# matter-labs/era-boojum

Measured on NVIDIA H100. Metric: goldilocks_ntt_gelements_per_s, higher is better.
Workload: dtype u64

## Files before the change

### era_boojum_b200/csrc/capi.cu

```cuda
#include <cstdlib>
#include <cstring>
#include <memory>
#include "ctx.hpp"

namespace bj {
int32_t poseidon2_init_constants(bj_ctx* ctx);
}

namespace bj {
__global__ void field_selftest_kernel(u64 n, u64 seed, unsigned long long* mismatches) {
  const u64 i = (u64)blockIdx.x * blockDim.x + threadIdx.x;
  if (i >= n) return;
  auto next = [](u64& s) {
    s += 0x9E3779B97F4A7C15ull;
    u64 z = s;
    z = (z ^ (z >> 30)) * 0xBF58476D1CE4E5B9ull;
    z = (z ^ (z >> 27)) * 0x94D049BB133111EBull;
    return z ^ (z >> 31);
  };
  u64 st = seed + i * 0x632BE59BD9B4E019ull;
  const u64 edges[12] = {0, 1, gl::P - 1, gl::P, gl::P + 1, ~0ull, gl::EPS, gl::EPS + 1, 1ull << 63, gl::P - gl::EPS, 2, gl::P - 2};
  u64 a = next(st), b = next(st);
  if ((i & 7) == 0) a = edges[(i >> 3) % 12];
  if ((i & 15) < 2) b = edges[(i >> 4) % 12];
// ... 2 lines not shown
    a = (1ull << ((i >> 3) & 63)) + (((i >> 9) & 3) == 1 ? 1 : 0) - (((i >> 9) & 3) == 2 ? 1 : 0);
    const unsigned sel = (unsigned)(i >> 11) & 7;
    u64 lo = r & 0xffffffffull, hi = r >> 32;
    if (sel & 1) lo = (sel & 4) ? 0xffffffffull : 0;
    if (sel & 2) hi = (sel & 4) ? 0xffffffffull : 0;
    b = (hi << 32) | lo;
  }
  if ((i & 63) == 5) {
    a = edges[(i >> 6) % 12];
    b = edges[(i >> 6) / 12 % 12];
  }
  unsigned bad = 0;
  if (gl::mul(a, b) != gl::mul_c(a, b)) bad++;
  if (gl::canon(gl::mul_lazy(a, b)) != gl::mul_c(a, b)) bad++;
  const u64 bc = gl::canon(b);
  if (gl::canon(gl::add(a, bc)) != gl::canon(gl::add_c(a, bc))) bad++;
  if (gl::canon(gl::sub(a, bc)) != gl::canon(gl::sub_c(a, bc))) bad++;
  if (gl::canon(gl::add(a, gl::P)) != gl::canon(a)) bad++;
  if (gl::canon(gl::sub(a, gl::P)) != gl::canon(a)) bad++;
  if (gl::mul(a, b) >= gl::P) bad++;
  if (bad) atomicAdd(mismatches, (unsigned long long)bad);
}
}

namespace bj {
static cudaMemPool_t private_pool(int device) {
  cudaMemPoolProps props = {};
  props.allocType = cudaMemAllocationTypePinned;
  props.handleTypes = cudaMemHandleTypeNone;
  props.location.type = cudaMemLocationTypeDevice;
  props.location.id = device;
  cudaMemPool_t pool = nullptr;
  if (cudaMemPoolCreate(&pool, &props) != cudaSuccess) {
    cudaGetLastError();
    return nullptr;
  }
  uint64_t keep = ~0ull;
  cudaMemPoolSetAttribute(pool, cudaMemPoolAttrReleaseThreshold, &keep);
  return pool;
}

int32_t ctx_new_lane(bj_ctx* parent, bj_ctx** out) {
  std::unique_ptr<bj_ctx> lane(new bj_ctx());
  lane->device = parent->device;
  lane->sm_count = parent->sm_count;
  lane->l2_persist_bytes = parent->l2_persist_bytes;
  lane->l2_window_max = parent->l2_window_max;
  lane->ntt_use_v2 = parent->ntt_use_v2;
  lane->ntt_col_fastest = parent->ntt_col_fastest;
  lane->ntt_max_tile_log = parent->ntt_max_tile_log;
  lane->ntt_pass1_w = parent->ntt_pass1_w;
  lane->ntt_chunk_mb = parent->ntt_chunk_mb;
  lane->ntt_full_pow = parent->ntt_full_pow;
  lane->gate_peephole = parent->gate_peephole;
  lane->gate_points_per_thread = parent->gate_points_per_thread;
  lane->ntt_l2_persist = 0;
  lane->ntt_bulk = parent->ntt_bulk;
  lane->memory_limit = parent->memory_limit;
  lane->allow_recompute_plan = parent->allow_recompute_plan;
  lane->max_row_blocks = parent->max_row_blocks;
  lane->own_twiddles = false;
  BJ_CUDA(parent, cudaStreamCreateWithFlags(&lane->stream, cudaStreamNonBlocking));
  lane->own_stream = true;
  lane->pool = private_pool(parent->device);
  {
    std::lock_guard<std::mutex> lock(parent->tables_mu);
    const cudaError_t e = cudaStreamSynchronize(parent->stream);
    if (e != cudaSuccess) {
      cudaStreamDestroy(lane->stream);
      if (lane->pool) cudaMemPoolDestroy(lane->pool);
      BJ_FAIL(parent, BJ_ERR_CUDA, std::string("bj_ctx_create_lane: cudaStreamSynchronize: ") + cudaGetErrorString(e));
    }
    lane->parent = parent;
    parent->lanes++;
  }
  *out = lane.release();
  return BJ_OK;
}
}

using namespace bj;

extern "C" {

int32_t bj_selftest_field(bj_ctx* ctx, uint64_t n, uint64_t seed, uint64_t* h_mismatches) {
  bj::DeviceGuard device_guard(ctx);
  if (!ctx || !h_mismatches) return BJ_ERR_INVALID_ARG;
  *h_mismatches = 0;
  if (n == 0) return BJ_OK;
  struct Counter {
    unsigned long long* d = nullptr;
    ~Counter() {
      if (d) cudaFree(d);
    }
  } c;
  BJ_CUDA(ctx, cudaMalloc(&c.d, sizeof(unsigned long long)));
  BJ_CUDA(ctx, cudaMemsetAsync(c.d, 0, sizeof(unsigned long long), ctx->stream));
  field_selftest_kernel<<<(unsigned)((n + 255) / 256), 256, 0, ctx->stream>>>(n, seed, c.d);
  BJ_LAUNCH_CHECK(ctx);
  unsigned long long h = 0;
  BJ_CUDA(ctx, cudaMemcpyAsync(&h, c.d, sizeof(h), cudaMemcpyDeviceToHost, ctx->stream));
  BJ_CUDA(ctx, cudaStreamSynchronize(ctx->stream));
  *h_mismatches = h;
  return BJ_OK;
}

// ... 2 lines not shown
const char* bj_status_string(int32_t s) {
  switch (s) {
    case BJ_OK: return "ok";
    case BJ_ERR_INVALID_ARG: return "invalid argument";
    case BJ_ERR_CUDA: return "CUDA error";
    case BJ_ERR_NO_DEVICE: return "no CUDA device (this library has no CPU fallback)";
    case BJ_ERR_OOM: return "out of device memory";
    case BJ_ERR_UNSUPPORTED: return "unsupported";
    default: return "unknown status";
  }
}

static int env_int(const char* name, int dflt) {
  const char* v = getenv(name);
  return v && *v ? atoi(v) : dflt;
}

int32_t bj_ctx_create(int32_t device, void* stream, bj_ctx** out_ctx) {
  if (!out_ctx) return BJ_ERR_INVALID_ARG;
  *out_ctx = nullptr;
  int count = 0;
  if (cudaGetDeviceCount(&count) != cudaSuccess || count == 0) {
    cudaGetLastError();
    return BJ_ERR_NO_DEVICE;
  }
  if (device < 0 || device >= count) return BJ_ERR_INVALID_ARG;
  bj_ctx* ctx = new bj_ctx();
  ctx->device = device;
  bj::DeviceGuard device_guard(ctx);
  {
    int cur = -1;
    if (cudaGetDevice(&cur) != cudaSuccess || cur != device) {
      cudaGetLastError();
      delete ctx;
      return BJ_ERR_CUDA;
    }
  }
  ctx->stream = (cudaStream_t)stream;
  cudaDeviceProp prop;
  if (cudaGetDeviceProperties(&prop, device) == cudaSuccess) {
    ctx->sm_count = prop.multiProcessorCount;
    ctx->l2_persist_bytes = std::min<size_t>((size_t)prop.l2CacheSize * 3 / 8, (size_t)prop.persistingL2CacheMaxSize);
    ctx->l2_window_max = (size_t)prop.accessPolicyMaxWindowSize;
  }
  ctx->ntt_max_tile_log = env_int("BJ_NTT_MAX_TILE_LOG", 13);
  ctx->gate_points_per_thread = env_int("BJ_GATE_POINTS_PER_THREAD", 0);
  ctx->gate_peephole = env_int("BJ_GATE_PEEPHOLE", 15);
  if (ctx->ntt_max_tile_log < 8) ctx->ntt_max_tile_log = 8;
  if (ctx->ntt_max_tile_log > 14) ctx->ntt_max_tile_log = 14;
  ctx->ntt_pass1_w = env_int("BJ_NTT_PASS1_W", -1);
  ctx->ntt_use_v2 = env_int("BJ_NTT_V2", 1);
  ctx->ntt_col_fastest = env_int("BJ_NTT_COL_FASTEST", -1);
  ctx->ntt_full_pow = env_int("BJ_NTT_FULL_POW", 1);
  ctx->ntt_bulk = env_int("BJ_NTT_BULK", 0);
  ctx->ntt_l2_persist = env_int("BJ_NTT_L2_PERSIST", 1);
  ctx->ntt_chunk_mb = env_int("BJ_NTT_CHUNK_MB", 0);
  ctx->pool = private_pool(device);
  int32_t st = poseidon2_init_constants(ctx);
  if (st != BJ_OK) {
    if (ctx->pool) cudaMemPoolDestroy(ctx->pool);
    delete ctx;
    return st;
  }
  *out_ctx = ctx;
  return BJ_OK;
}

int32_t bj_ctx_destroy(bj_ctx* ctx) {
  if (!ctx) return BJ_OK;
  bj::DeviceGuard device_guard(ctx);
  if (const uint32_t alive = ctx->lanes.load())
    BJ_FAIL(ctx, BJ_ERR_INVALID_ARG, "bj_ctx_destroy: " + std::to_string(alive) + " lane(s) of this context are alive: destroy them first");
  if (ctx->parent) {
    std::lock_guard<std::mutex> lock(ctx->parent->tables_mu);
    if (ctx->witness_sets)
      BJ_FAIL(ctx, BJ_ERR_INVALID_ARG, "bj_ctx_destroy: " + std::to_string(ctx->witness_sets) + " witness slot set(s) of this lane are alive: free them first");
  }
  cudaStreamSynchronize(ctx->stream);
  if (ctx->witness_stream) {
    cudaStreamSynchronize(ctx->witness_stream);
    cudaStreamDestroy(ctx->witness_stream);
  }
  if (ctx->own_twiddles) {
    if (ctx->tw_fwd) cudaFree(ctx->tw_fwd);
    if (ctx->tw_inv) cudaFree(ctx->tw_inv);
  }
  for (auto& e : ctx->pow_cache) {
    cudaFree(e.lo);
    cudaFree(e.hi);
    if (e.full) cudaFree(e.full);
  }
  for (void* p : ctx->tables_retired) cudaFree(p);
  if (ctx->pow_best) cudaFree(ctx->pow_best);
  if (ctx->gate_program) cudaFree(ctx->gate_program);
  if (ctx->pool) cudaMemPoolDestroy(ctx->pool);
  if (ctx->scratch) cudaFree(ctx->scratch);
  if (ctx->ptr_table) cudaFree(ctx->ptr_table);
  if (ctx->param_arena) cudaFree(ctx->param_arena);
  if (ctx->host_ring) cudaFree(ctx->host_ring);
  if (ctx->copy_streams_ready) {
    cudaStreamDestroy(ctx->h2d_stream);
    cudaStreamDestroy(ctx->d2h_stream);
    for (int i = 0; i < 3; i++) {
      cudaEventDestroy(ctx->ev_up[i]);
      cudaEventDestroy(ctx->ev_done[i]);
      cudaEventDestroy(ctx->ev_down[i]);
    }
  }
  if (ctx->own_stream) cudaStreamDestroy(ctx->stream);
  if (ctx->parent) {
    std::lock_guard<std::mutex> lock(ctx->parent->tables_mu);
    ctx->parent->lanes--;
  }
  delete ctx;
  return BJ_OK;
}

int32_t bj_ctx_set_stream(bj_ctx* ctx, void* stream) {
  bj::DeviceGuard device_guard(ctx);
  if (!ctx) return BJ_ERR_INVALID_ARG;
  if (ctx->parent) BJ_FAIL(ctx, BJ_ERR_INVALID_ARG, "bj_ctx_set_stream: a lane keeps the stream it was created with");
  BJ_CUDA(ctx, cudaStreamSynchronize(ctx->stream));
  ctx->stream = (cudaStream_t)stream;
  return BJ_OK;
}

int32_t bj_ctx_set_coset_shard(bj_ctx* ctx, uint32_t rank, uint32_t world, uint32_t log_lde) {
  bj::DeviceGuard device_guard(ctx);
  if (!ctx) return BJ_ERR_INVALID_ARG;
  if (world == 0 || (world & (world - 1)) || rank >= world || log_lde > 16 || world > (1u << log_lde))
    BJ_FAIL(ctx, BJ_ERR_INVALID_ARG, "bj_ctx_set_coset_shard: world must be a power of two <= the LDE factor and rank < world");
  uint32_t ls = 0;
  while ((1u << ls) < world) ls++;
  ctx->shard_log_lde = log_lde;
  ctx->shard.first = rank;
  ctx->shard.log_stride = ls;
  ctx->shard.log_split = 0;
  return BJ_OK;
}

int32_t bj_ctx_set_domain_shard(bj_ctx* ctx, uint32_t rank, uint32_t world, uint32_t log_lde) {
  bj::DeviceGuard device_guard(ctx);
  if (!ctx) return BJ_ERR_INVALID_ARG;
  if (world == 0 || (world & (world - 1)) || rank >= world || log_lde > 16 || world > (8u << log_lde))
// ... 124 lines not shown
```

### era_boojum_b200/csrc/ctx.hpp

```cpp
#pragma once
#include <cuda_runtime.h>
#include <stdint.h>
#include <algorithm>
#include <atomic>
#include <mutex>
#include <string>
#include <vector>
#include "../../include/boojum_b200.h"
#include "gl64.cuh"

namespace bj {
using gl::u64;
using gl::u32;

struct PowTab {
  u64 coset;
  int log_n;
  u64 scale;
  int split;
  u64* lo;
  u64* hi;
  u64* full;
};

struct CosetShard {
  uint32_t first = 0;
  uint32_t log_stride = 0;
  uint32_t log_split = 0;
  __host__ __device__ __forceinline__ u64 global_index(u64 t_loc, int log_coset_len) const {
    if (log_stride == 0) return t_loc;
    const int lu = log_coset_len - (int)log_split;
    const u64 i = t_loc & ((1ull << lu) - 1);
    const u64 k = t_loc >> lu;
    return ((((k << log_stride) | first)) << lu) | i;
  }
  __host__ __device__ __forceinline__ u64 unit_of(u64 rank, u64 k) const { return (k << log_stride) | rank; }
  __host__ __device__ __forceinline__ u64 global_unit(u64 k) const { return unit_of(first, k); }
  __host__ __device__ __forceinline__ u64 local_units(u64 cosets) const {
    const u64 stride = 1ull << log_stride, group = cosets << log_split;
    if (group >= stride) return group >> log_stride;
    return first < group ? 1 : 0;
  }
  __host__ __device__ __forceinline__ u64 local_points(u64 cosets, int log_coset_len) const {
    return local_units(cosets) << (log_coset_len - (int)log_split);
  }
  __host__ __device__ __forceinline__ u32 owner(u64 t, int log_coset_len) const {
    return (u32)((t >> (log_coset_len - (int)log_split)) & ((1ull << log_stride) - 1));
  }
  __host__ __device__ __forceinline__ u64 owner_index(u64 t, int log_coset_len) const {
    const int lu = log_coset_len - (int)log_split;
    return (((t >> lu) >> log_stride) << lu) | (t & ((1ull << lu) - 1));
  }
  __host__ u64 unit_shift(u64 u, u32 log_n, u32 log_lde) const {
    const u64 j = u >> log_split, p = u & ((1ull << log_split) - 1);
    u64 jr = 0, pr = 0;
    for (u32 b = 0; b < log_lde; b++) jr |= ((j >> b) & 1) << (log_lde - 1 - b);
    for (u32 b = 0; b < log_split; b++) pr |= ((p >> b) & 1) << (log_split - 1 - b);
    u64 s = gl::mul(gl::MULT_GEN, gl::pow(gl::omega(log_n + log_lde), jr));
    if (log_split) s = gl::mul(s, gl::pow(gl::omega(log_n), pr));
    return s;
  }
  __host__ static CosetShard window(uint32_t log_units, uint32_t u, uint32_t log_split = 0) {
    CosetShard w;
    w.first = u;
    w.log_stride = log_units;
    w.log_split = log_split;
    return w;
  }
};

}

struct bj_comm;

struct bj_ctx {
  int device = 0;
  bj_comm* comm = nullptr;
  cudaStream_t stream = nullptr;
  bool own_stream = false;
  std::string last_error;
  bj::u64* tw_fwd = nullptr;
  bj::u64* tw_inv = nullptr;
  int tw_log = 0;
  std::vector<bj::PowTab> pow_cache;
  size_t pow_full_bytes = 0;
  void* scratch = nullptr;
  size_t scratch_bytes = 0;
  void* ptr_table = nullptr;
  size_t ptr_table_bytes = 0;
  bool copy_streams_ready = false;
  cudaStream_t h2d_stream = nullptr, d2h_stream = nullptr;
  cudaEvent_t ev_up[3] = {}, ev_done[3] = {}, ev_down[3] = {};
  void* host_ring = nullptr;
  size_t host_ring_bytes = 0;
  cudaStream_t witness_stream = nullptr;
  uint32_t witness_sets = 0;
  uint64_t witness_set_bytes = 0;
  uint32_t lane_witness_sets = 0;
  uint64_t lane_witness_set_bytes = 0;
  void* param_arena = nullptr;
  size_t param_off = 0;
  uint64_t launches = 0;
  int sm_count = 132;
  bool ntt_attr_set = false;
  std::vector<void*> attr_done;
  int ntt_use_v2 = 1;
  int ntt_col_fastest = -1;
  int ntt_max_tile_log = 13;
  int ntt_pass1_w = -1;
  int ntt_chunk_mb = 0;
  int ntt_full_pow = 1;
  uint32_t one = 1;
  int gate_peephole = 15;
  int gate_points_per_thread = 0;
  int ntt_l2_persist = 1;
  bool l2_limit_set = false;
  size_t l2_persist_bytes = 0;
  size_t l2_window_max = 0;
  int ntt_bulk = 0;
  cudaMemPool_t pool = nullptr;
  bj::CosetShard shard;
  uint32_t shard_log_lde = 0;
  uint64_t memory_limit = 0;
  bool allow_recompute_plan = false;
  bool allow_sharded_recompute_plan = false;
  uint32_t max_row_blocks = 1;
  unsigned long long* pow_best = nullptr;
  void* gate_program = nullptr;
  size_t gate_program_bytes = 0;
  bj_ctx* parent = nullptr;
  std::atomic<uint32_t> lanes{0};
  std::mutex tables_mu;
  std::vector<void*> tables_retired;
  bool own_twiddles = true;
  std::vector<const bj_setup*> setups;
};

#define BJ_FAIL(ctx, code, msg)          \
  do {                                   \
    if (ctx) (ctx)->last_error = (msg);  \
    return (code);                       \
  } while (0)

#define BJ_CUDA(ctx, expr)                                                                      \
  do {                                                                                          \
    cudaError_t _e = (expr);                                                                    \
    if (_e != cudaSuccess) {                                                                    \
      if (ctx) (ctx)->last_error = std::string(#expr) + ": " + cudaGetErrorString(_e);          \
      return BJ_ERR_CUDA;                                                                       \
    }                                                                                           \
  } while (0)

#define BJ_TRY(expr)                 \
  do {                               \
    int32_t _s = (expr);             \
    if (_s != BJ_OK) return _s;      \
  } while (0)

#define BJ_LAUNCH_CHECK(ctx)                                                              \
  do {                                                                                    \
    (ctx)->launches++;                                                                    \
    cudaError_t _e = cudaGetLastError();                                                  \
    if (_e != cudaSuccess) {                                                              \
      (ctx)->last_error = std::string("kernel launch: ") + cudaGetErrorString(_e);        \
// ... 35 lines not shown
```

### era_boojum_b200/csrc/ntt.cu

```cuda
#include <algorithm>
#include <cstdlib>
#include "ctx.hpp"
#include "ntt.cuh"
#include "ntt_v2.cuh"

namespace bj {

using gl::u32;

__device__ __forceinline__ int phys(int e) { return e + (e >> 4); }

__device__ __forceinline__ u64 scale_factor(const NttPass& p, u64 idx) {
  if (p.scale_mode == SCALE_CONST) return p.scale_const;
  if (p.scale_mode == SCALE_FULL) return __ldg(p.pw_full + idx);
  u64 lo = __ldg(p.pw_lo + (idx & ((1ull << p.pw_split) - 1)));
  u64 hi = __ldg(p.pw_hi + (idx >> p.pw_split));
  return gl::mul(lo, hi);
}

template <int RS>
__device__ __forceinline__ void stage_compute(u64 (&x)[16], const u64* __restrict__ tab, u32 pfx) {
#pragma unroll
  for (int q = 0; q < RS; q++) {
    const int bit = 1 << (3 - q);
// ... 9 lines not shown
    }
  }
}

__global__ void __launch_bounds__(512) ntt_pass_kernel(const NttPass p) {
  extern __shared__ u64 sm[];
  const int t = p.t, w = p.w, LOG_E = t + w;
  const int E = 1 << LOG_E, W = 1 << w;
  const int tid = threadIdx.x, nthr = blockDim.x;
  const u64 tile = blockIdx.x;
  const u64* __restrict__ src = p.src + (u64)blockIdx.y * p.src_col_stride;
  u64* __restrict__ dst = p.dst + (u64)blockIdx.y * p.dst_col_stride;
  const int m = p.log_n, r0 = p.r0;
  const bool do_scale = p.scale_mode != SCALE_NONE;

  u64 base = 0, S = 1;
  u32 hi = 0;
  if (p.kind == PASS_TILE) {
    const int lo_bits = m - r0 - t;
    const int groups_log = lo_bits - w;
    S = 1ull << lo_bits;
    hi = (u32)(tile >> groups_log);
    const u64 lo0 = (tile & ((1ull << groups_log) - 1)) << w;
    base = ((u64)hi << (m - r0)) + lo0;
    for (int e = tid; e < E; e += nthr) {
      const int row = e >> w, col = e & (W - 1);
      const u64 gi = base + (u64)row * S + col;
      u64 v = src[gi];
      if (do_scale && p.scale_on_load) v = gl::mul(v, scale_factor(p, gi));
      sm[phys(e)] = v;
    }
  } else {
    for (int idx = tid; idx < E; idx += nthr) {
      const int col = idx >> t, row = idx & ((1 << t) - 1);
      const u32 k1 = (u32)(tile << w) + col;
      const u32 blk = r0 ? (__brev(k1) >> (32 - r0)) : 0u;
      const u64 gi = ((u64)blk << t) + row;
      u64 v = src[gi];
      if (do_scale && p.scale_on_load) v = gl::mul(v, scale_factor(p, gi));
      sm[phys(row * W + col)] = v;
    }
  }
  __syncthreads();

  int done = 0;
  int rs = t & 3;
  if (rs == 0) rs = 4;
  const int nvt = E >> 4;
  while (done < t) {
    const int b_lo = t - done - rs;
    const int pp = b_lo + w - (4 - rs);
    for (int q = tid; q < nvt; q += nthr) {
      const int e0 = ((q >> pp) << (pp + 4)) | (q & ((1 << pp) - 1));
      u32 hq = hi;
      if (p.kind != PASS_TILE) {
        const u32 k1 = (u32)(tile << w) + (e0 & (W - 1));
        hq = r0 ? (__brev(k1) >> (32 - r0)) : 0u;
      }
      const u32 pfx = (hq << (LOG_E - pp - 4)) | (u32)(q >> pp);
      u64 x[16];
#pragma unroll
      for (int j = 0; j < 16; j++) x[j] = sm[phys(e0 | (j << pp))];
      switch (rs) {
        case 1: stage_compute<1>(x, p.tab, pfx); break;
        case 2: stage_compute<2>(x, p.tab, pfx); break;
        case 3: stage_compute<3>(x, p.tab, pfx); break;
        default: stage_compute<4>(x, p.tab, pfx); break;
      }
#pragma unroll
      for (int j = 0; j < 16; j++) sm[phys(e0 | (j << pp))] = x[j];
    }
    __syncthreads();
    done += rs;
    rs = 4;
  }

  if (p.kind == PASS_TILE) {
    for (int e = tid; e < E; e += nthr) {
      const int row = e >> w, col = e & (W - 1);
      const u64 gi = base + (u64)row * S + col;
      u64 v = sm[phys(e)];
      if (do_scale && !p.scale_on_load) v = gl::mul(v, scale_factor(p, gi));
      if (p.canon_out) v = gl::canon(v);
      dst[gi] = v;
    }
  } else {
    for (int idx = tid; idx < E; idx += nthr) {
      const int col = idx & (W - 1);
      const u32 kappa = (u32)(idx >> w);
      const u32 rho = t ? (__brev(kappa) >> (32 - t)) : 0u;
      u64 v = sm[phys((int)rho * W + col)];
      const u64 k1 = (tile << w) + col;
      const u64 go = k1 + ((u64)kappa << r0);
      if (do_scale && !p.scale_on_load) v = gl::mul(v, scale_factor(p, go));
      if (p.canon_out) v = gl::canon(v);
      dst[go] = v;
    }
  }
}

__global__ void ntt_small_kernel(u64* data, u64 col_stride, u32 n_cols, int log_n, const u64* __restrict__ tab,
                                 u64 coset_or_inv, u64 n_inv, int inverse) {
  const u32 c = blockIdx.x * blockDim.x + threadIdx.x;
  if (c >= n_cols) return;
  u64* a = data + (u64)c * col_stride;
  const int n = 1 << log_n;
  u64 x[8];
// ... 4 lines not shown
      x[i] = gl::mul(x[i], s);
      s = gl::mul(s, coset_or_inv);
    }
  }
  int pairs = n / 2, groups = 1, dist = n / 2;
  while (groups < n) {
    for (int k = 0; k < groups; k++) {
      const u64 s = tab[k];
      for (int j = k * pairs * 2; j < k * pairs * 2 + pairs; j++) {
        const u64 u = x[j], v = gl::mul(x[j + dist], s);
        x[j + dist] = gl::canon(gl::sub(u, v));
        x[j] = gl::canon(gl::add(u, v));
      }
    }
    pairs /= 2;
    groups *= 2;
    dist /= 2;
  }
  if (inverse) {
    u64 y[8];
    for (int i = 0; i < n; i++) y[log_n ? (__brev((u32)i) >> (32 - log_n)) : 0] = x[i];
    u64 s = n_inv;
    for (int i = 0; i < n; i++) {
      x[i] = gl::mul(y[i], s);
      s = gl::mul(s, coset_or_inv);
    }
  }
  for (int i = 0; i < n; i++) a[i] = gl::canon(x[i]);
}

struct PowSquares {
  u64 sq[33];
};

__global__ void twiddle_table_kernel(u64* tab, u32 count, int bits, PowSquares ps) {
  const u32 k = blockIdx.x * blockDim.x + threadIdx.x;
  if (k >= count) return;
  const u32 e = bits ? (__brev(k) >> (32 - bits)) : 0u;
  u64 r = 1;
  for (int b = 0; b < bits; b++)
    if ((e >> b) & 1) r = gl::mul(r, ps.sq[b]);
  tab[k] = gl::canon(r);
}

__global__ void pow_table_kernel(u64* out, u32 count, int bits, PowSquares ps, u64 scale) {
  const u32 i = blockIdx.x * blockDim.x + threadIdx.x;
  if (i >= count) return;
  u64 r = scale;
  for (int b = 0; b < bits; b++)
    if ((i >> b) & 1) r = gl::mul(r, ps.sq[b]);
  out[i] = gl::canon(r);
}

__global__ void bitreverse_kernel(u64* data, u64 col_stride, int log_n) {
  const u64 i = (u64)blockIdx.x * blockDim.x + threadIdx.x;
  if (i >= (1ull << log_n)) return;
  u64* a = data + (u64)blockIdx.y * col_stride;
  const u64 j = __brevll(i) >> (64 - log_n);
  if (i < j) {
    const u64 t = a[i];
    a[i] = a[j];
    a[j] = t;
  }
}


int32_t ensure_scratch(bj_ctx* ctx, size_t bytes) {
  if (ctx->scratch_bytes >= bytes) return BJ_OK;
  if (ctx->scratch) {
    BJ_CUDA(ctx, cudaStreamSynchronize(ctx->stream));
    BJ_CUDA(ctx, cudaFree(ctx->scratch));
    ctx->scratch = nullptr;
    ctx->scratch_bytes = 0;
  }
  cudaError_t e = cudaMalloc(&ctx->scratch, bytes);
  if (e != cudaSuccess) {
    cudaGetLastError();
    BJ_FAIL(ctx, BJ_ERR_OOM, "scratch allocation failed");
  }
  ctx->scratch_bytes = bytes;
  return BJ_OK;
}

static PowSquares make_squares(u64 w) {
  PowSquares ps;
  for (int b = 0; b < 33; b++) {
    ps.sq[b] = w;
    w = gl::sqr(w);
  }
  return ps;
}

static int32_t release_retired(bj_ctx* owner) {
  if (owner->tables_retired.empty() || owner->lanes.load() > 0) return BJ_OK;
  BJ_CUDA(owner, cudaStreamSynchronize(owner->stream));
  for (void* p : owner->tables_retired) cudaFree(p);
  owner->tables_retired.clear();
  owner->pow_full_bytes = 0;
  for (const auto& e : owner->pow_cache)
    if (e.full) owner->pow_full_bytes += sizeof(u64) << e.log_n;
  return BJ_OK;
}

int32_t ensure_twiddles(bj_ctx* ctx, int log_n) {
  if (log_n < 1) log_n = 1;
  if (log_n > 32) BJ_FAIL(ctx, BJ_ERR_INVALID_ARG, "log_n > 32 (two-adicity of the field)");
  if (ctx->tw_log >= log_n) return BJ_OK;
  if (ctx->parent && !ctx->own_twiddles) {
    bj_ctx* p = ctx->parent;
    std::lock_guard<std::mutex> lock(p->tables_mu);
    if (p->tw_log >= log_n) {
      ctx->tw_fwd = p->tw_fwd;
      ctx->tw_inv = p->tw_inv;
      ctx->tw_log = p->tw_log;
      return BJ_OK;
    }
    ctx->tw_fwd = ctx->tw_inv = nullptr;
    ctx->tw_log = 0;
    ctx->own_twiddles = true;
  }
  std::unique_lock<std::mutex> lock(ctx->tables_mu, std::defer_lock);
  if (!ctx->parent) {
    lock.lock();
    BJ_TRY(release_retired(ctx));
  }
  if (ctx->tw_fwd) {
    BJ_CUDA(ctx, cudaStreamSynchronize(ctx->stream));
    if (ctx->lanes.load() > 0) {
      ctx->tables_retired.push_back(ctx->tw_fwd);
      ctx->tables_retired.push_back(ctx->tw_inv);
    } else {
      cudaFree(ctx->tw_fwd);
      cudaFree(ctx->tw_inv);
    }
    ctx->tw_fwd = ctx->tw_inv = nullptr;
    ctx->tw_log = 0;
  }
  const u32 count = 1u << (log_n - 1);
  u64 *fwd = nullptr, *inv = nullptr;
  BJ_CUDA(ctx, cudaMalloc(&fwd, sizeof(u64) * count));
  BJ_CUDA(ctx, cudaMalloc(&inv, sizeof(u64) * count));
  const u64 w = gl::omega(log_n);
  const u32 blocks = (count + 255) / 256;
  twiddle_table_kernel<<<blocks, 256, 0, ctx->stream>>>(fwd, count, log_n - 1, make_squares(w));
  BJ_LAUNCH_CHECK(ctx);
  twiddle_table_kernel<<<blocks, 256, 0, ctx->stream>>>(inv, count, log_n - 1, make_squares(gl::inv(w)));
  BJ_LAUNCH_CHECK(ctx);
  if (ctx->lanes.load() > 0) BJ_CUDA(ctx, cudaStreamSynchronize(ctx->stream));
  ctx->tw_fwd = fwd;
  ctx->tw_inv = inv;
  ctx->tw_log = log_n;
  return BJ_OK;
}

__global__ void __launch_bounds__(256) pow_full_kernel(u64* __restrict__ full, u64 n, const u64* __restrict__ lo,
                                                        const u64* __restrict__ hi, int split) {
  const u64 i = (u64)blockIdx.x * blockDim.x + threadIdx.x;
  if (i >= n) return;
  full[i] = gl::mul(__ldg(lo + (i & ((1ull << split) - 1))), __ldg(hi + (i >> split)));
}

static constexpr size_t POW_FULL_BUDGET = (size_t)3 << 30;
static int32_t get_pow_tables(bj_ctx* ctx, u64 c, int log_n, u64 scale, PowTab* out) {
  bj_ctx* owner = ctx->parent ? ctx->parent : ctx;
  std::lock_guard<std::mutex> lock(owner->tables_mu);
  if (owner == ctx) BJ_TRY(release_retired(ctx));
  for (auto& e : owner->pow_cache)
    if (e.coset == c && e.log_n == log_n && e.scale == scale) {
      *out = e;
      return BJ_OK;
    }
  const bool shared = owner->lanes.load() > 0;
  if (owner->pow_cache.size() >= 64) {
    BJ_CUDA(ctx, cudaStreamSynchronize(ctx->stream));
    for (auto& e : owner->pow_cache) {
      if (shared) {
        owner->tables_retired.insert(owner->tables_retired.end(), {(void*)e.lo, (void*)e.hi});
        if (e.full) owner->tables_retired.push_back(e.full);
        continue;
      }
      cudaFree(e.lo);
      cudaFree(e.hi);
      if (e.full) cudaFree(e.full);
    }
    owner->pow_cache.clear();
    if (!shared) owner->pow_full_bytes = 0;
  }
  PowTab pt;
  pt.coset = c;
  pt.log_n = log_n;
  pt.scale = scale;
  pt.split = log_n / 2;
  const u32 nlo = 1u << pt.split, nhi = 1u << (log_n - pt.split);
  BJ_CUDA(ctx, cudaMalloc(&pt.lo, sizeof(u64) * nlo));
  BJ_CUDA(ctx, cudaMalloc(&pt.hi, sizeof(u64) * nhi));
  pow_table_kernel<<<(nlo + 255) / 256, 256, 0, ctx->stream>>>(pt.lo, nlo, pt.split, make_squares(c), 1);
  BJ_LAUNCH_CHECK(ctx);
  const u64 chi = gl::pow(c, 1ull << pt.split);
  pow_table_kernel<<<(nhi + 255) / 256, 256, 0, ctx->stream>>>(pt.hi, nhi, log_n - pt.split, make_squares(chi),
                                                                gl::canon(scale));
  BJ_LAUNCH_CHECK(ctx);
  pt.full = nullptr;
  const size_t full_bytes = sizeof(u64) << log_n;
  if (ctx->ntt_full_pow && log_n >= 8 && owner->pow_full_bytes + full_bytes <= POW_FULL_BUDGET &&
      cudaMalloc(&pt.full, full_bytes) == cudaSuccess) {
    const u64 n = 1ull << log_n;
    pow_full_kernel<<<(unsigned)((n + 255) / 256), 256, 0, ctx->stream>>>(pt.full, n, pt.lo, pt.hi, pt.split);
    BJ_LAUNCH_CHECK(ctx);
    owner->pow_full_bytes += full_bytes;
  } else {
    cudaGetLastError();
    pt.full = nullptr;
  }
  if (shared) BJ_CUDA(ctx, cudaStreamSynchronize(ctx->stream));
  owner->pow_cache.push_back(pt);
  *out = pt;
  return BJ_OK;
}

int32_t get_pow_tables_public(bj_ctx* ctx, u64 c, int log_n, u64 scale, PowTab* out) { return get_pow_tables(ctx, c, log_n, scale, out); }

static constexpr int NTT_MAX_PASSES = 6;

struct Plan {
  int n_pass;
  int t[NTT_MAX_PASSES];
  int w[NTT_MAX_PASSES];
};

static bool make_plan(const bj_ctx* ctx, int m, bool transpose_last, Plan* out) {
  Plan& pl = *out;
  pl = Plan{};
  const int MAXE = ctx->ntt_max_tile_log;
  if (m <= 12) {
    pl.n_pass = 1;
    pl.t[0] = m;
    pl.w[0] = 0;
    return true;
  }
  const int TL = transpose_last ? MAXE - 2 : MAXE;
  const int TM = MAXE - 2;
  int t_last = std::min(TL, std::max((m + 1) / 2, m - 10));
  int rest = m - t_last;
  int n_front = (rest + TM - 1) / TM;
  pl.n_pass = n_front + 1;
  if (pl.n_pass > NTT_MAX_PASSES) return false;
  int r0 = 0;
  for (int i = 0; i < n_front; i++) {
    int ti = rest / (n_front - i);
    rest -= ti;
    int wi = ctx->ntt_pass1_w >= 0 ? ctx->ntt_pass1_w : std::max(2, std::min(5, MAXE - ti));
    wi = std::min(wi, MAXE - ti);
    wi = std::min(wi, m - r0 - ti);
    if (ti + wi < 4) wi = 4 - ti;
    pl.t[i] = ti;
    pl.w[i] = wi;
    r0 += ti;
  }
  pl.t[n_front] = t_last;
  pl.w[n_front] = transpose_last ? std::min(std::min(MAXE - t_last, 5), r0) : 0;
  return true;
}

static constexpr u32 MAX_GRID_Y = 65535;

template <typename F>
static int32_t launch_column_slices(bj_ctx* ctx, const NttPass& p, u32 n_cols, F&& fn) {
  for (u32 c0 = 0; c0 < n_cols; c0 += std::min(MAX_GRID_Y, n_cols - c0)) {
    NttPass ps = p;
    ps.src = p.src + (u64)c0 * p.src_col_stride;
    ps.dst = p.dst + (u64)c0 * p.dst_col_stride;
    fn(ps, std::min(MAX_GRID_Y, n_cols - c0));
    BJ_LAUNCH_CHECK(ctx);
  }
// ... 23 lines not shown
    bool col_fastest;
    if (ctx->ntt_col_fastest >= 0) {
      col_fastest = (ctx->ntt_col_fastest >> (is_last ? 1 : 0)) & 1;
    } else {
      const bool big_table = p.scale_mode == SCALE_FULL && (sizeof(u64) << p.log_n) > ctx->l2_persist_bytes;
      col_fastest = is_last || big_table;
    }
    if (p.kind == PASS_TILE && !bulk && col_fastest && tiles * n_cols <= 0x7fffffffull) {
      NttPass ps = p;
      ps.n_cols = n_cols;
      v2.fn<<<(unsigned)(tiles * n_cols), v2.threads, v2.smem, ctx->stream>>>(ps);
      BJ_LAUNCH_CHECK(ctx);
      return BJ_OK;
    }
    return launch_column_slices(ctx, p, n_cols, [&](const NttPass& ps, u32 cols) {
      v2.fn<<<dim3((unsigned)tiles, cols, 1), v2.threads, v2.smem, ctx->stream>>>(ps);
    });
  }
  const int threads = std::max(32, std::min(512, (1 << LOG_E) >> 4));
  const size_t smem = sizeof(u64) * ((size_t)(1 << LOG_E) + ((size_t)(1 << LOG_E) >> 4) + 1);
  if (!ctx->ntt_attr_set) {
    BJ_CUDA(ctx, cudaFuncSetAttribute(ntt_pass_kernel, cudaFuncAttributeMaxDynamicSharedMemorySize, 200 * 1024));
    BJ_CUDA(ctx, cudaFuncSetAttribute(ntt_pass_kernel, cudaFuncAttributePreferredSharedMemoryCarveout,
                                      cudaSharedmemCarveoutMaxShared));
    ctx->ntt_attr_set = true;
  }
  return launch_column_slices(ctx, p, n_cols, [&](const NttPass& ps, u32 cols) {
    ntt_pass_kernel<<<dim3((unsigned)tiles, cols, 1), threads, smem, ctx->stream>>>(ps);
  });
}

static int32_t run_transform(bj_ctx* ctx, const u64* src, u64 src_stride, u64* dst, u64 dst_stride, int m,
                             u32 n_cols, u64 coset, bool inverse, u64* scratch, u64 scratch_stride) {
  BJ_TRY(ensure_twiddles(ctx, m));
  const u64* tab = inverse ? ctx->tw_inv : ctx->tw_fwd;
  coset = gl::canon(coset);
  if (m < 4) {
    if (src != dst || src_stride != dst_stride) {
      for (u32 c = 0; c < n_cols; c++)
        BJ_CUDA(ctx, cudaMemcpyAsync(dst + c * dst_stride, src + c * src_stride, sizeof(u64) << m,
                                     cudaMemcpyDeviceToDevice, ctx->stream));
    }
    const u64 n_inv = gl::inv((u64)1 << m);
    ntt_small_kernel<<<(n_cols + 63) / 64, 64, 0, ctx->stream>>>(dst, dst_stride, n_cols, m, tab,
                                                                 inverse ? gl::inv(coset) : coset, n_inv, inverse);
    BJ_LAUNCH_CHECK(ctx);
    return BJ_OK;
  }
  Plan pl;
  if (!make_plan(ctx, m, inverse, &pl)) BJ_FAIL(ctx, BJ_ERR_UNSUPPORTED, "NTT plan needs more passes than NTT_MAX_PASSES");
  PowTab pt{};
  int scale_mode = SCALE_NONE;
  u64 scale_const = 1;
  if (!inverse) {
    if (coset != 1) {
      BJ_TRY(get_pow_tables(ctx, coset, m, 1, &pt));
      scale_mode = SCALE_POW;
    }
  } else {
    const u64 n_inv = gl::inv((u64)1 << m);
    if (coset != 1) {
      BJ_TRY(get_pow_tables(ctx, gl::inv(coset), m, n_inv, &pt));
      scale_mode = SCALE_POW;
    } else {
      scale_mode = SCALE_CONST;
      scale_const = n_inv;
    }
  }
  const u64* cur_src = src;
  u64 cur_src_stride = src_stride;
  int r0 = 0;
  for (int i = 0; i < pl.n_pass; i++) {
    const bool first = i == 0, last = i == pl.n_pass - 1;
    NttPass p{};
    p.tab = tab;
    p.log_n = m;
    p.r0 = r0;
    p.t = pl.t[i];
    p.w = pl.w[i];
    p.kind = (inverse && last) ? PASS_TRANSPOSE_LAST : PASS_TILE;
    p.src = cur_src;
    p.src_col_stride = cur_src_stride;
    if (inverse && pl.n_pass > 1) {
      const int remaining = pl.n_pass - 1 - i;
      const bool to_dst = (remaining % 2) == 0;
      p.dst = to_dst ? dst : scratch;
      p.dst_col_stride = to_dst ? dst_stride : scratch_stride;
      if (last && p.dst == p.src) BJ_FAIL(ctx, BJ_ERR_INVALID_ARG, "internal: in-place transpose pass");
    } else {
      p.dst = dst;
      p.dst_col_stride = dst_stride;
    }
    p.scale_mode = SCALE_NONE;
    if (!inverse && first && scale_mode != SCALE_NONE) {
      p.scale_mode = scale_mode;
      p.scale_on_load = 1;
    }
    if (inverse && last) {
      p.scale_mode = scale_mode;
      p.scale_on_load = 0;
      p.scale_const = scale_const;
    }
    p.pw_lo = pt.lo;
    p.pw_hi = pt.hi;
    p.pw_split = pt.split;
    p.pw_full = pt.full;
    if (p.scale_mode == SCALE_POW && pt.full) p.scale_mode = SCALE_FULL;
    p.canon_out = last ? 1 : 0;
    const bool pin = ctx->ntt_l2_persist && p.scale_mode == SCALE_FULL && n_cols > 1 && ctx->l2_persist_bytes && ctx->l2_window_max;
    if (pin) {
      if (!ctx->l2_limit_set) {
        cudaDeviceSetLimit(cudaLimitPersistingL2CacheSize, ctx->l2_persist_bytes);
        cudaGetLastError();
        ctx->l2_limit_set = true;
      }
      cudaStreamAttrValue av = {};
      av.accessPolicyWindow.base_ptr = (void*)p.pw_full;
      av.accessPolicyWindow.num_bytes = std::min<size_t>(sizeof(u64) << m, ctx->l2_window_max);
      av.accessPolicyWindow.hitRatio = std::min(1.0f, (float)ctx->l2_persist_bytes / (float)av.accessPolicyWindow.num_bytes);
      av.accessPolicyWindow.hitProp = cudaAccessPropertyPersisting;
      av.accessPolicyWindow.missProp = cudaAccessPropertyStreaming;
      if (cudaStreamSetAttribute(ctx->stream, cudaStreamAttributeAccessPolicyWindow, &av) != cudaSuccess) cudaGetLastError();
    }
    const int32_t st_pass = launch_pass(ctx, p, n_cols);
    if (pin) {
      cudaStreamAttrValue av = {};
      av.accessPolicyWindow.num_bytes = 0;
      if (cudaStreamSetAttribute(ctx->stream, cudaStreamAttributeAccessPolicyWindow, &av) != cudaSuccess) cudaGetLastError();
// ... 269 lines not shown
```

### era_boojum_b200/csrc/ntt.cuh

```cuda
#pragma once
#include "gl64.cuh"

namespace bj {

using gl::u64;

enum NttScaleMode : int { SCALE_NONE = 0, SCALE_CONST = 1, SCALE_POW = 2, SCALE_FULL = 3 };
enum NttPassKind : int { PASS_TILE = 0, PASS_TRANSPOSE_LAST = 1 };

struct NttPass {
  const u64* src;
  u64* dst;
  u64 src_col_stride;
  u64 dst_col_stride;
  const u64* tab;
  int log_n;
  int r0;
  int t;
  int w;
  int kind;
  int scale_mode;
  int scale_on_load;
  u64 scale_const;
  const u64* pw_lo;
  const u64* pw_hi;
  int pw_split;
  const u64* pw_full;
  int canon_out;
  unsigned n_cols;
};

}
```

### era_boojum_b200/csrc/ntt_v2.cuh

```cuda
#pragma once
#include "ntt.cuh"

#ifndef BJ_NTT_ADD_ALU
#define BJ_NTT_ADD_ALU 0
#endif
#ifndef BJ_NTT_SUB_FMA
#define BJ_NTT_SUB_FMA 0
#endif

namespace bj {

using gl::u32;

template <int T, int W>
struct V2Cfg {
  static constexpr int LOG_E = T + W;
  static constexpr int E = 1 << LOG_E;
  static constexpr int NVT = E >> 4;
  static constexpr int THREADS = NVT < 32 ? 32 : (NVT > 256 ? 256 : NVT);
  static constexpr int RS0 = (T & 3) ? (T & 3) : 4;
  static constexpr int NSTAGES = (T + 3) / 4;
  static constexpr size_t SMEM = sizeof(u64) * (size_t)(E + (E >> 4) + 2);
  static constexpr bool CAP_REGS = (T == 12 && W == 0);
};
// ... 112 lines not shown
  const bool scale_store = p.scale_mode != SCALE_NONE && !p.scale_on_load;

  u64 base = 0;
  int lo_bits = 0;
  u32 hi = 0;
  if constexpr (KIND == PASS_TILE) {
    lo_bits = m - r0 - T;
    const int groups_log = lo_bits - W;
    hi = tile >> groups_log;
    const u64 lo0 = (u64)(tile & ((1u << groups_log) - 1)) << W;
    base = ((u64)hi << (m - r0)) + lo0;
#pragma unroll 4
    for (int pi = tid; pi < C::E / 2; pi += C::THREADS) {
      const int e = 2 * pi;
      const int row = e >> W, col = e & WM;
      const u64 gi = base + ((u64)row << lo_bits) + col;
      ulonglong2 v;
      if constexpr (W == 0) {
        v = *reinterpret_cast<const ulonglong2*>(src + base + e);
      } else {
        v = *reinterpret_cast<const ulonglong2*>(src + gi);
      }
      if (scale_load) {
        const u64 g0 = (W == 0) ? base + e : gi;
        u64 s0, s1;
        v2_scale2(p, g0, s0, s1);
        v.x = gl::mul(v.x, s0);
        v.y = gl::mul(v.y, s1);
      }
      const int pe = v2_phys(e);
      sm[pe] = v.x;
      sm[pe + 1] = v.y;
    }
  } else {
#pragma unroll 4
    for (int pi = tid; pi < C::E / 2; pi += C::THREADS) {
      const int col = pi >> (T - 1), row = (pi & ((1 << (T - 1)) - 1)) * 2;
      const u32 k1 = (tile << W) + col;
      const u32 blk = r0 ? (__brev(k1) >> (32 - r0)) : 0u;
      const u64 gi = ((u64)blk << T) + row;
      ulonglong2 v = *reinterpret_cast<const ulonglong2*>(src + gi);
      if (scale_load) {
        u64 s0, s1;
        v2_scale2(p, gi, s0, s1);
        v.x = gl::mul(v.x, s0);
        v.y = gl::mul(v.y, s1);
      }
      sm[v2_phys((row << W) + col)] = v.x;
      sm[v2_phys(((row + 1) << W) + col)] = v.y;
    }
  }
  __syncthreads();

  if (r0 == 0) v2_stage<T, W, KIND, 0, true>(sm, p.tab, tid, hi, tile, r0);
  else v2_stage<T, W, KIND, 0, false>(sm, p.tab, tid, hi, tile, r0);

  if constexpr (KIND == PASS_TILE) {
#pragma unroll 4
    for (int pi = tid; pi < C::E / 2; pi += C::THREADS) {
      const int e = 2 * pi;
      const int row = e >> W, col = e & WM;
      const u64 gi = (W == 0) ? base + e : base + ((u64)row << lo_bits) + col;
      const int pe = v2_phys(e);
      ulonglong2 v;
      v.x = sm[pe];
      v.y = sm[pe + 1];
      if (scale_store) {
        u64 s0, s1;
        v2_scale2(p, gi, s0, s1);
        v.x = gl::mul(v.x, s0);
        v.y = gl::mul(v.y, s1);
      }
      if (p.canon_out) {
        v.x = gl::canon(v.x);
        v.y = gl::canon(v.y);
      }
      *reinterpret_cast<ulonglong2*>(dst + gi) = v;
    }
  } else if constexpr (W == 0) {
#pragma unroll 4
    for (int kappa = tid; kappa < C::E; kappa += C::THREADS) {
      const u32 rho = __brev((u32)kappa) >> (32 - T);
      u64 v = sm[v2_phys((int)rho)];
      const u64 go = (u64)tile + ((u64)kappa << r0);
      if (scale_store) v = gl::mul(v, v2_scale(p, go));
      if (p.canon_out) v = gl::canon(v);
      dst[go] = v;
    }
  } else {
#pragma unroll 4
    for (int pi = tid; pi < C::E / 2; pi += C::THREADS) {
      const int col = (pi & (WM >> 1)) * 2;
      const u32 kappa = (u32)(pi >> (W - 1));
      const u32 rho = __brev(kappa) >> (32 - T);
      const int pe = v2_phys(((int)rho << W) + col);
      ulonglong2 v;
      v.x = sm[pe];
      v.y = sm[pe + 1];
      const u64 go = ((u64)tile << W) + col + ((u64)kappa << r0);
      if (scale_store) {
        u64 s0, s1;
        v2_scale2(p, go, s0, s1);
        v.x = gl::mul(v.x, s0);
        v.y = gl::mul(v.y, s1);
      }
      if (p.canon_out) {
        v.x = gl::canon(v.x);
        v.y = gl::canon(v.y);
// ... 4 lines not shown
}

template <int T, int W, int KIND>
__global__ void __launch_bounds__(V2Cfg<T, W>::THREADS) ntt_pass_v2_kernel(const NttPass p) {
  ntt_pass_v2_body<T, W, KIND>(p);
}
template <int T, int W, int KIND>
__global__ void __launch_bounds__(V2Cfg<T, W>::THREADS, 3) ntt_pass_v2_kernel_r85(const NttPass p) {
  ntt_pass_v2_body<T, W, KIND>(p);
}
template <int T, int W, int KIND>
__global__ void __launch_bounds__(V2Cfg<T, W>::THREADS, 4) ntt_pass_v2_kernel_r64(const NttPass p) {
  ntt_pass_v2_body<T, W, KIND>(p);
}

__device__ __forceinline__ u32 smem_u32(const void* p) { return (u32)__cvta_generic_to_shared(p); }

template <int T>
__global__ void __launch_bounds__(V2Cfg<T, 0>::THREADS) ntt_pass_bulk_kernel(const NttPass p) {
  using C = V2Cfg<T, 0>;
  extern __shared__ __align__(128) u64 sm[];
  constexpr int PADDED = (C::E + (C::E >> 4) + 2 + 15) & ~15;
  u64* stage = sm + PADDED;
  __shared__ __align__(8) unsigned long long bar;
  const int tid = threadIdx.x;
  const u32 tile = blockIdx.x;
  const u64* __restrict__ src = p.src + (u64)blockIdx.y * p.src_col_stride + ((u64)tile << T);
  u64* __restrict__ dst = p.dst + (u64)blockIdx.y * p.dst_col_stride + ((u64)tile << T);
  constexpr u32 BYTES = (u32)(sizeof(u64) << T);
  if (tid == 0) {
    asm volatile("mbarrier.init.shared::cta.b64 [%0], 1;" ::"r"(smem_u32(&bar)));
    asm volatile("fence.mbarrier_init.release.cluster;" ::: "memory");
  }
  __syncthreads();
  if (tid == 0) {
    asm volatile("mbarrier.arrive.expect_tx.shared::cta.b64 _, [%0], %1;" ::"r"(smem_u32(&bar)), "r"(BYTES) : "memory");
    asm volatile("cp.async.bulk.shared::cluster.global.mbarrier::complete_tx::bytes [%0], [%1], %2, [%3];" ::"r"(smem_u32(stage)), "l"(src),
                 "r"(BYTES), "r"(smem_u32(&bar))
                 : "memory");
  }
  {
    u32 done = 0;
    while (!done)
      asm volatile("{\n\t.reg .pred q;\n\tmbarrier.try_wait.parity.shared::cta.b64 q, [%1], 0;\n\tselp.u32 %0, 1, 0, q;\n\t}" : "=r"(done) : "r"(smem_u32(&bar)) : "memory");
  }
#pragma unroll 4
  for (int pi = tid; pi < C::E / 2; pi += C::THREADS) {
    const ulonglong2 v = reinterpret_cast<const ulonglong2*>(stage)[pi];
    const int pe = v2_phys(2 * pi);
    sm[pe] = v.x;
    sm[pe + 1] = v.y;
  }
  __syncthreads();
  if (p.r0 == 0) v2_stage<T, 0, PASS_TILE, 0, true>(sm, p.tab, tid, tile, tile, p.r0);
  else v2_stage<T, 0, PASS_TILE, 0, false>(sm, p.tab, tid, tile, tile, p.r0);
#pragma unroll 4
  for (int pi = tid; pi < C::E / 2; pi += C::THREADS) {
    const int pe = v2_phys(2 * pi);
    ulonglong2 v;
    v.x = sm[pe];
    v.y = sm[pe + 1];
    if (p.canon_out) {
      v.x = gl::canon(v.x);
      v.y = gl::canon(v.y);
    }
    reinterpret_cast<ulonglong2*>(stage)[pi] = v;
  }
  asm volatile("fence.proxy.async.shared::cta;" ::: "memory");
  __syncthreads();
  if (tid == 0) {
    asm volatile("cp.async.bulk.global.shared::cta.bulk_group [%0], [%1], %2;" ::"l"(dst), "r"(smem_u32(stage)), "r"(BYTES) : "memory");
    asm volatile("cp.async.bulk.commit_group;" ::: "memory");
    asm volatile("cp.async.bulk.wait_group.read 0;" ::: "memory");
  }
}

template <int T>
struct V2BulkCfg {
  static constexpr size_t SMEM = sizeof(u64) * (size_t)(((V2Cfg<T, 0>::E + (V2Cfg<T, 0>::E >> 4) + 2 + 15) & ~15) + V2Cfg<T, 0>::E);
};

typedef void (*V2KernelPtr)(const NttPass);

template <int T, int W, int KIND>
struct V2Entry {
  static V2KernelPtr get() {
    if constexpr (V2Cfg<T, W>::CAP_REGS) return ntt_pass_v2_kernel_r64<T, W, KIND>;
    else if constexpr (T + W == 13) return ntt_pass_v2_kernel_r85<T, W, KIND>;
    else return ntt_pass_v2_kernel<T, W, KIND>;
  }
};

struct V2Launch {
  V2KernelPtr fn;
  int threads;
  size_t smem;
};

#define BJ_V2_CASE(TT, WW)                                                                   \
  if (t == TT && w == WW) {                                                                  \
    out->fn = kind == PASS_TILE ? V2Entry<TT, WW, PASS_TILE>::get()                          \
                                : V2Entry<TT, WW, PASS_TRANSPOSE_LAST>::get();                \
    out->threads = V2Cfg<TT, WW>::THREADS;                                                   \
    out->smem = V2Cfg<TT, WW>::SMEM;                                                         \
    return true;                                                                             \
  }

static bool v2_bulk_lookup(int t, V2Launch* out) {
// ... 24 lines not shown
```

Measured before the change: 37.84.

## Fold coset scaling into precomputed twisted twiddle table for forward NTT

For forward coset NTTs above a size threshold, a cached per-coset twisted twiddle table is built. Each entry is the original twiddle multiplied by the matching power of the coset. Passes then index this table through a prefix bit instead of scaling elements with the power tables on load. This removes the per-element coset multiplication and its pow-table lookups, at the cost of extra device memory per coset/size and a one-time build kernel.

```diff
diff --git a/era_boojum_b200/csrc/capi.cu b/era_boojum_b200/csrc/capi.cu
--- a/era_boojum_b200/csrc/capi.cu
+++ b/era_boojum_b200/csrc/capi.cu
@@ -78,6 +78,7 @@
   lane->ntt_pass1_w = parent->ntt_pass1_w;
   lane->ntt_chunk_mb = parent->ntt_chunk_mb;
   lane->ntt_full_pow = parent->ntt_full_pow;
+  lane->ntt_twist = parent->ntt_twist;
   lane->gate_peephole = parent->gate_peephole;
   lane->gate_points_per_thread = parent->gate_points_per_thread;
   lane->ntt_l2_persist = 0;
@@ -186,6 +187,7 @@
   ctx->ntt_use_v2 = env_int("BJ_NTT_V2", 1);
   ctx->ntt_col_fastest = env_int("BJ_NTT_COL_FASTEST", -1);
   ctx->ntt_full_pow = env_int("BJ_NTT_FULL_POW", 1);
+  ctx->ntt_twist = env_int("BJ_NTT_TWIST", 1);
   ctx->ntt_bulk = env_int("BJ_NTT_BULK", 0);
   ctx->ntt_l2_persist = env_int("BJ_NTT_L2_PERSIST", 1);
   ctx->ntt_chunk_mb = env_int("BJ_NTT_CHUNK_MB", 0);
@@ -224,6 +226,7 @@
     cudaFree(e.hi);
     if (e.full) cudaFree(e.full);
   }
+  for (auto& e : ctx->twist_cache) cudaFree(e.tab);
   for (void* p : ctx->tables_retired) cudaFree(p);
   if (ctx->pow_best) cudaFree(ctx->pow_best);
   if (ctx->gate_program) cudaFree(ctx->gate_program);
diff --git a/era_boojum_b200/csrc/ctx.hpp b/era_boojum_b200/csrc/ctx.hpp
--- a/era_boojum_b200/csrc/ctx.hpp
+++ b/era_boojum_b200/csrc/ctx.hpp
@@ -23,6 +23,12 @@
   u64* full;
 };
 
+struct TwistTab {
+  u64 coset;
+  int log_n;
+  u64* tab;
+};
+
 struct CosetShard {
   uint32_t first = 0;
   uint32_t log_stride = 0;
@@ -83,6 +89,7 @@
   bj::u64* tw_inv = nullptr;
   int tw_log = 0;
   std::vector<bj::PowTab> pow_cache;
+  std::vector<bj::TwistTab> twist_cache;
   size_t pow_full_bytes = 0;
   void* scratch = nullptr;
   size_t scratch_bytes = 0;
@@ -110,6 +117,7 @@
   int ntt_pass1_w = -1;
   int ntt_chunk_mb = 0;
   int ntt_full_pow = 1;
+  int ntt_twist = 1;
   uint32_t one = 1;
   int gate_peephole = 15;
   int gate_points_per_thread = 0;
diff --git a/era_boojum_b200/csrc/ntt.cu b/era_boojum_b200/csrc/ntt.cu
--- a/era_boojum_b200/csrc/ntt.cu
+++ b/era_boojum_b200/csrc/ntt.cu
@@ -85,7 +85,7 @@
     const int pp = b_lo + w - (4 - rs);
     for (int q = tid; q < nvt; q += nthr) {
       const int e0 = ((q >> pp) << (pp + 4)) | (q & ((1 << pp) - 1));
-      u32 hq = hi;
+      u32 hq = hi | p.tw_prefix;
       if (p.kind != PASS_TILE) {
         const u32 k1 = (u32)(tile << w) + (e0 & (W - 1));
         hq = r0 ? (__brev(k1) >> (32 - r0)) : 0u;
@@ -196,6 +196,17 @@
   out[i] = gl::canon(r);
 }
 
+__global__ void twist_table_kernel(u64* tw, u32 count, int log_n, const u64* __restrict__ tab, PowSquares ps) {
+  const u32 i = blockIdx.x * blockDim.x + threadIdx.x;
+  if (i >= count) return;
+  if (i == 0) {
+    tw[0] = 0;
+    return;
+  }
+  const int r = 31 - __clz(i);
+  tw[i] = gl::canon(gl::mul(__ldg(tab + (i - (1u << r))), ps.sq[log_n - r - 1]));
+}
+
 __global__ void bitreverse_kernel(u64* data, u64 col_stride, int log_n) {
   const u64 i = (u64)blockIdx.x * blockDim.x + threadIdx.x;
   if (i >= (1ull << log_n)) return;
@@ -235,14 +246,20 @@
   return ps;
 }
 
+static size_t cached_full_bytes(const bj_ctx* owner) {
+  size_t b = 0;
+  for (const auto& e : owner->pow_cache)
+    if (e.full) b += sizeof(u64) << e.log_n;
+  for (const auto& e : owner->twist_cache) b += sizeof(u64) << e.log_n;
+  return b;
+}
+
 static int32_t release_retired(bj_ctx* owner) {
   if (owner->tables_retired.empty() || owner->lanes.load() > 0) return BJ_OK;
   BJ_CUDA(owner, cudaStreamSynchronize(owner->stream));
   for (void* p : owner->tables_retired) cudaFree(p);
   owner->tables_retired.clear();
-  owner->pow_full_bytes = 0;
-  for (const auto& e : owner->pow_cache)
-    if (e.full) owner->pow_full_bytes += sizeof(u64) << e.log_n;
+  owner->pow_full_bytes = cached_full_bytes(owner);
   return BJ_OK;
 }
 
@@ -328,7 +345,7 @@
       if (e.full) cudaFree(e.full);
     }
     owner->pow_cache.clear();
-    if (!shared) owner->pow_full_bytes = 0;
+    if (!shared) owner->pow_full_bytes = cached_full_bytes(owner);
   }
   PowTab pt;
   pt.coset = c;
@@ -364,6 +381,43 @@
 
 int32_t get_pow_tables_public(bj_ctx* ctx, u64 c, int log_n, u64 scale, PowTab* out) { return get_pow_tables(ctx, c, log_n, scale, out); }
 
+static constexpr int TWIST_MIN_LOG = 13;
+static int32_t get_twist_table(bj_ctx* ctx, u64 c, int log_n, const u64** out) {
+  *out = nullptr;
+  bj_ctx* owner = ctx->parent ? ctx->parent : ctx;
+  std::lock_guard<std::mutex> lock(owner->tables_mu);
+  if (owner == ctx) BJ_TRY(release_retired(ctx));
+  for (const auto& e : owner->twist_cache)
+    if (e.coset == c && e.log_n == log_n) {
+      *out = e.tab;
+      return BJ_OK;
+    }
+  const bool shared = owner->lanes.load() > 0;
+  if (owner->twist_cache.size() >= 64) {
+    BJ_CUDA(ctx, cudaStreamSynchronize(ctx->stream));
+    for (auto& e : owner->twist_cache) {
+      if (shared) owner->tables_retired.push_back(e.tab);
+      else cudaFree(e.tab);
+    }
+    owner->twist_cache.clear();
+    if (!shared) owner->pow_full_bytes = cached_full_bytes(owner);
+  }
+  const size_t bytes = sizeof(u64) << log_n;
+  TwistTab tt{c, log_n, nullptr};
+  if (owner->pow_full_bytes + bytes > POW_FULL_BUDGET || cudaMalloc(&tt.tab, bytes) != cudaSuccess) {
+    cudaGetLastError();
+    return BJ_OK;
+  }
+  const u32 count = 1u << log_n;
+  twist_table_kernel<<<(count + 255) / 256, 256, 0, ctx->stream>>>(tt.tab, count, log_n, ctx->tw_fwd, make_squares(c));
+  BJ_LAUNCH_CHECK(ctx);
+  owner->pow_full_bytes += bytes;
+  if (shared) BJ_CUDA(ctx, cudaStreamSynchronize(ctx->stream));
+  owner->twist_cache.push_back(tt);
+  *out = tt.tab;
+  return BJ_OK;
+}
+
 static constexpr int NTT_MAX_PASSES = 6;
 
 struct Plan {
@@ -493,8 +547,10 @@
   PowTab pt{};
   int scale_mode = SCALE_NONE;
   u64 scale_const = 1;
+  const u64* twist = nullptr;
   if (!inverse) {
-    if (coset != 1) {
+    if (coset != 1 && ctx->ntt_twist && ctx->ntt_full_pow && m >= TWIST_MIN_LOG) BJ_TRY(get_twist_table(ctx, coset, m, &twist));
+    if (coset != 1 && !twist) {
       BJ_TRY(get_pow_tables(ctx, coset, m, 1, &pt));
       scale_mode = SCALE_POW;
     }
@@ -514,7 +570,8 @@
   for (int i = 0; i < pl.n_pass; i++) {
     const bool first = i == 0, last = i == pl.n_pass - 1;
     NttPass p{};
-    p.tab = tab;
+    p.tab = twist ? twist : tab;
+    p.tw_prefix = twist ? 1u << r0 : 0u;
     p.log_n = m;
     p.r0 = r0;
     p.t = pl.t[i];
diff --git a/era_boojum_b200/csrc/ntt.cuh b/era_boojum_b200/csrc/ntt.cuh
--- a/era_boojum_b200/csrc/ntt.cuh
+++ b/era_boojum_b200/csrc/ntt.cuh
@@ -27,6 +27,7 @@
   int pw_split;
   const u64* pw_full;
   int canon_out;
+  unsigned tw_prefix;
   unsigned n_cols;
 };
 
diff --git a/era_boojum_b200/csrc/ntt_v2.cuh b/era_boojum_b200/csrc/ntt_v2.cuh
--- a/era_boojum_b200/csrc/ntt_v2.cuh
+++ b/era_boojum_b200/csrc/ntt_v2.cuh
@@ -188,8 +188,10 @@
   }
   __syncthreads();
 
-  if (r0 == 0) v2_stage<T, W, KIND, 0, true>(sm, p.tab, tid, hi, tile, r0);
-  else v2_stage<T, W, KIND, 0, false>(sm, p.tab, tid, hi, tile, r0);
+  const u32 tw_prefix = KIND == PASS_TILE ? p.tw_prefix : 0u;
+  const u32 hs = hi | tw_prefix;
+  if ((r0 | tw_prefix) == 0) v2_stage<T, W, KIND, 0, true>(sm, p.tab, tid, hs, tile, r0);
+  else v2_stage<T, W, KIND, 0, false>(sm, p.tab, tid, hs, tile, r0);
 
   if constexpr (KIND == PASS_TILE) {
 #pragma unroll 4
@@ -300,8 +302,8 @@
     sm[pe + 1] = v.y;
   }
   __syncthreads();
-  if (p.r0 == 0) v2_stage<T, 0, PASS_TILE, 0, true>(sm, p.tab, tid, tile, tile, p.r0);
-  else v2_stage<T, 0, PASS_TILE, 0, false>(sm, p.tab, tid, tile, tile, p.r0);
+  if ((p.r0 | p.tw_prefix) == 0) v2_stage<T, 0, PASS_TILE, 0, true>(sm, p.tab, tid, tile, tile, p.r0);
+  else v2_stage<T, 0, PASS_TILE, 0, false>(sm, p.tab, tid, tile | p.tw_prefix, tile, p.r0);
 #pragma unroll 4
   for (int pi = tid; pi < C::E / 2; pi += C::THREADS) {
     const int pe = v2_phys(2 * pi);
```

After: 41.68 (median of 6 runs). 10.2% higher.
